# rchikhi/rust-seq2kminmers

Hardware: AMD Instinct MI355X
Metric: input bases/s (Gbp/s) for k-min-mer extraction, l=31 k=10 d=0.01 (higher is better)
Workload: dtype u32

## Files before the change

### rust-seq2kminmers_amd/csrc/s2k_tile_impl.h

```cpp
#pragma once
#include "s2k_dev.h"
#include "s2k_static_l.h"

#include <cstdlib>
#include <mutex>
#include <type_traits>

namespace s2k {
namespace {

#ifndef S2K_TW
#define S2K_TW 12
#endif
#ifndef S2K_TW_REG
#ifdef S2K_PROFILE
#define S2K_TW_REG 12
#else
#define S2K_TW_REG 16
#endif
#endif
template <bool HPC> constexpr int tw() { return HPC ? S2K_TW : S2K_TW_REG; }
template <bool HPC> constexpr int waves_per_simd() { return tw<HPC>() / 4; }
static_assert(S2K_TW % 4 == 0 && S2K_TW_REG % 4 == 0, "whole waves per SIMD");
constexpr int HS_OFF = 16;
constexpr int BUF_BYTES = HS_OFF + TILE_BASES + 128;
#ifndef S2K_CAPP
#define S2K_CAPP 16
#endif
constexpr int CAPP = S2K_CAPP;
constexpr int NPC = TILE_T / CAPP;
constexpr int MAX_L_TILED = 64;
#ifndef S2K_LISTCAP
#define S2K_LISTCAP 256
#endif
#ifndef S2K_JOBCAP
#define S2K_JOBCAP 32
#endif
#ifndef S2K_REDERIVE_GROUP
#define S2K_REDERIVE_GROUP 8
#endif
constexpr int LISTCAP_REG = S2K_TW_REG > 12 ? 216 : S2K_LISTCAP;
constexpr int LISTCAP_HPC = 192;
template <bool HPC> constexpr int listcap() { return HPC ? LISTCAP_HPC : LISTCAP_REG; }
template <bool HPC> constexpr int jobcap() { return !HPC && S2K_TW_REG > 12 ? 16 : S2K_JOBCAP; }
#ifndef S2K_REG_LA
#define S2K_REG_LA 1
#endif
#ifndef S2K_HPC_LA
#define S2K_HPC_LA 2
#endif
constexpr int REG_LA = S2K_REG_LA;
constexpr int HPC_LA = S2K_HPC_LA;
constexpr int NBL = 32;
template <bool DESC> constexpr int stores_per_round() { return DESC ? 1 : 3; }
static_assert(NBL == META_SEGS, "TileMeta keeps NBL segment starts");
constexpr int NPRE = 10;

#ifndef S2K_SD_SHIFT
#define S2K_SD_SHIFT 6
#endif
constexpr int ROW_W = 6, ROW_PFX = 4, ROW_CUM = 5, N_ROWS = 66, SD_SHIFT = S2K_SD_SHIFT;
struct HpcLds {
    uint32_t row[N_ROWS][ROW_W];
    uint32_t halo_pos[64];
    uint8_t sd[SD_SHIFT == 6 ? 160 : 288];
};
static_assert(sizeof(HpcLds) % 16 == 0, "the tile buffer behind it is read 16 bytes at a time");
struct NoHpcLds {};

template <bool HPC>
struct alignas(16) WaveLdsT : std::conditional<HPC, HpcLds, NoHpcLds>::type {
    uint8_t buf[BUF_BYTES];
    uint16_t list[listcap<HPC>()];
    uint16_t jobx[jobcap<HPC>()];
    uint16_t jobslot[jobcap<HPC>()];
    int16_t hb[NBL];
    uint16_t rs16[NBL];
};
#ifdef S2K_PROFILE
typedef __attribute__((address_space(3))) unsigned long long *ph_ptr_t;
constexpr int PROFILE_LDS_BYTES = 16 * 16 * 8;
#else
typedef uint64_t *ph_ptr_t;
constexpr int PROFILE_LDS_BYTES = 0;
#endif
constexpr int SEED_TABLE_BYTES = 2 * 256 * 8;
#ifndef S2K_SEL8
#define S2K_SEL8 1
#endif
constexpr int TABLE_BYTES = SEED_TABLE_BYTES;
constexpr int SEL8_OFF = SEED_TABLE_BYTES, SEL8_BYTES = S2K_SEL8 ? 256 * 8 : 0;
#ifndef S2K_PASS2_ACC
#define S2K_PASS2_ACC 1
#endif
static_assert(!S2K_PASS2_ACC || S2K_SEL8, "pass 2 reads its v_perm_b32 selectors from sel8");
#ifndef S2K_LPH
#define S2K_LPH 0
#endif
#ifndef S2K_WARM2
#define S2K_WARM2 1
#endif
constexpr int WARM_OFF = SEL8_OFF + SEL8_BYTES, WARM_BYTES = S2K_WARM2 ? 256 * 8 : 0;
template <bool HPC> constexpr int table_bytes() { return SEED_TABLE_BYTES + (HPC ? SEL8_BYTES + WARM_BYTES : 0); }
template <bool HPC>
constexpr int block_lds_bytes() { return table_bytes<HPC>() + tw<HPC>() * (int)sizeof(WaveLdsT<HPC>) + PROFILE_LDS_BYTES; }
#ifndef S2K_EXPERIMENT
static_assert(block_lds_bytes<true>() <= 160 * 1024 && block_lds_bytes<false>() <= 160 * 1024, "the block of a CU must fit its 160 KiB of LDS");
#endif

__device__ inline uint32_t wave_incl_scan(uint32_t v, int lane) {
    (void)lane;
    uint32_t t;
    t = (uint32_t)__builtin_amdgcn_update_dpp(0, (int)v, 0x111, 0xf, 0xf, false);
    uint32_t a = v + t;
    t = (uint32_t)__builtin_amdgcn_update_dpp(0, (int)v, 0x112, 0xf, 0xf, false);
    a += t;
    t = (uint32_t)__builtin_amdgcn_update_dpp(0, (int)v, 0x113, 0xf, 0xf, false);
    a += t;
    t = (uint32_t)__builtin_amdgcn_update_dpp(0, (int)a, 0x114, 0xf, 0xe, false);
    a += t;
    t = (uint32_t)__builtin_amdgcn_update_dpp(0, (int)a, 0x118, 0xf, 0xc, false);
    a += t;
// ... 320 lines not shown
#ifdef S2K_ISA_MARKS
#define S2K_STAMP(i) do { (void)ph; (void)stamp; asm volatile("; S2K_PHASE %0" ::"i"(i)); } while (0)
#else
#define S2K_STAMP(i) do { (void)ph; (void)stamp; } while (0)
#endif
#endif

template <class WL>
__device__ __forceinline__ uint32_t hpc_compact(uint8_t *D, WL &S, const uint8_t *__restrict__ bases,
                                                const uint64_t *__restrict__ read_off, uint64_t n_reads, uint64_t n_bases,
                                                uint64_t t0, uint32_t tile_len, uint32_t r0, uint32_t r1, uint32_t l,
                                                int lane, uint32_t &halo_n_out, uint64_t bpos0,
                                                uint32_t prev_byte0, bool forced0, const Sem &sem, ph_ptr_t ph,
                                                uint64_t &stamp) {
    typedef __attribute__((address_space(3))) uint8_t lds_u8;
    {
        uint64_t sp = bpos0;
        for (uint64_t c0 = 0;; c0 += 64) {
            if (sp > t0 && sp < t0 + tile_len) {
                const uint32_t rel = (uint32_t)(sp - t0), o = div_tile_t(rel), i = rel - __umul24(o, (uint32_t)TILE_T);
                atomicOr(&S.row[o][i >> 5], 1u << (i & 31u));
            }
            if ((uint64_t)r0 + 1 + c0 + 64 > (uint64_t)r1) break;
            const uint64_t ri = (uint64_t)r0 + 1 + c0 + 64 + lane;
            sp = ri <= n_reads ? read_off[ri] : ~0ull;
            __builtin_amdgcn_s_waitcnt(0x0F70);
        }
    }
    wave_sync();
    S2K_STAMP(13);
    uint32_t c[36];
    const uint32_t lane_off = __umul24((uint32_t)TILE_T, (uint32_t)lane);
    const uint4 *src = reinterpret_cast<const uint4 *>(D + lane_off);
#pragma unroll
    for (int p = 0; p < 9; p++) {
        uint4 v = src[p];
        c[4 * p] = v.x; c[4 * p + 1] = v.y; c[4 * p + 2] = v.z; c[4 * p + 3] = v.w;
    }
    uint32_t fmk[5];
    {
        const uint2 *rr = reinterpret_cast<const uint2 *>(&S.row[lane][0]);
        const uint2 r01 = rr[0], r23 = rr[1];
        fmk[0] = r01.x; fmk[1] = r01.y; fmk[2] = r23.x; fmk[3] = r23.y;
        fmk[4] = S.row[lane][4];
    }
    if (lane == 0 && forced0) fmk[0] |= 1u;
    const uint32_t prevw = (uint32_t)__builtin_amdgcn_update_dpp((int)(prev_byte0 << 24), (int)c[35], 0x138, 0xf, 0xf, false);
    const uint32_t last_raw = bcast(c[35] >> 24, 63);
    const uint32_t la_a = D[TILE_BASES + lane], la_b = D[TILE_BASES + 64 + lane];
    const int vb = (int)tile_len - (int)lane_off;
    const bool partial = tile_len < (uint32_t)TILE_BASES;
    uint32_t pr[4];
#pragma unroll
    for (int d = 0; d < 36; d++) {
        const uint32_t cur = c[d];
        const uint32_t prv = __builtin_amdgcn_alignbyte(cur, d == 0 ? prevw : c[d - 1], 3);
        uint32_t x;
        asm("v_bitop3_b32 %0, %1, %2, %3 bitop3:0x96" : "=v"(x) : "v"(cur), "v"(prv), "v"(0x0C0C0C0Cu));
        const uint32_t y = __builtin_amdgcn_perm(0xFFFFFFFFu, 0xFFFFFFFFu, x);
        const int j = (d & 7) >> 1;
        if ((d & 1) == 0) pr[j] = __builtin_amdgcn_udot4(y, 0x08040201u, 255u, false);
        else pr[j] = __builtin_amdgcn_udot4(y, 0x80402010u, pr[j], false);
        if (d == 35) fmk[4] |= __builtin_amdgcn_perm(pr[1], pr[0], 0x0C0C0501u);
        else if ((d & 7) == 7)
            fmk[d >> 3] |= __builtin_amdgcn_perm(pr[1], pr[0], 0x0C0C0501u) | __builtin_amdgcn_perm(pr[3], pr[2], 0x05010C0Cu);
    }
    if (partial) {
#pragma unroll
        for (int g = 0; g < 5; g++) {
            const int v = vb - 32 * g;
            fmk[g] &= v >= 32 ? 0xFFFFFFFFu : (v <= 0 ? 0u : ((1u << v) - 1u));
        }
    }
    const uint32_t p0 = __popc(fmk[0]), p1 = p0 + __popc(fmk[1]), p2 = p1 + __popc(fmk[2]), p3 = p2 + __popc(fmk[3]);
    uint32_t cnt = p3 + __popc(fmk[4]);
    uint32_t incl = wave_incl_scan(cnt, lane);
    uint32_t base = incl - cnt;
    const uint32_t R = bcast(incl, 63);
    {
        uint2 *rw = reinterpret_cast<uint2 *>(&S.row[lane][0]);
        rw[0] = make_uint2(fmk[0], fmk[1]);
        rw[1] = make_uint2(fmk[2], fmk[3]);
        rw[2] = make_uint2(fmk[4] | (base << 16), p0 | (p1 << 8) | (p2 << 16) | (p3 << 24));
        if (lane < N_ROWS - 64) *reinterpret_cast<uint2 *>(&S.row[64 + lane][ROW_PFX]) = make_uint2(R << 16, 0u);
        if (cnt)
            for (uint32_t m = (base + (1u << SD_SHIFT) - 1u) >> SD_SHIFT; (m << SD_SHIFT) < base + cnt; m++) S.sd[m] = (uint8_t)lane;
    }
    wave_sync();
    S2K_STAMP(14);
#if S2K_PASS2_ACC
    {
        typedef __attribute__((address_space(3))) const unsigned long long *lds_cu64;
        uint4 *zp = reinterpret_cast<uint4 *>(D + lane_off);
#pragma unroll
        for (int p = 0; p < 9; p++) zp[p] = make_uint4(0, 0, 0, 0);
        asm volatile("" ::: "memory");
        const uint32_t(&fmk_)[5] = fmk;
        auto pass2 = [&](auto sparse_c) {
            constexpr bool SPARSE = decltype(sparse_c)::value;
            uint32_t fm[5] = {fmk_[0], fmk_[1], fmk_[2], fmk_[3], fmk_[4]};
#pragma unroll
            for (int g = 0; g < 5; g++) asm volatile("" : "+v"(fm[g]));
            if constexpr (!SPARSE) {
                uint32_t qa = (uint32_t)(uintptr_t)(lds_u8 *)D + base - 1u, carry = 0;
#pragma unroll
                for (int q0 = 0; q0 < 18; q0 += 9) {
                    unsigned long long e[9];
                    uint32_t ix[9];
#pragma unroll
                    for (int qq = 0; qq < 9; qq++) {
                        ix[qq] = byte_x8_sel(fm[(q0 + qq) >> 2], (q0 + qq) & 3);
                        e[qq] = *reinterpret_cast<lds_cu64>((uint32_t)SEL8_OFF + ix[qq]);
                    }
#pragma unroll
                    for (int qq = 0; qq < 9; qq++) {
                        const int q = q0 + qq;
                        const uint32_t plo = __builtin_amdgcn_perm(c[2 * q + 1], c[2 * q], (uint32_t)e[qq]);
                        const uint32_t phi = __builtin_amdgcn_perm(c[2 * q + 1], c[2 * q], (uint32_t)(e[qq] >> 32));
                        const uint32_t sh = ~qa, waddr = qa & ~3u;
                        const uint32_t w0 = __builtin_amdgcn_alignbyte(plo, 0u, sh) | carry, w1 = __builtin_amdgcn_alignbyte(phi, plo, sh);
                        carry = __builtin_amdgcn_alignbyte(0u, phi, sh);
                        asm volatile("ds_or_b32 %0, %1\n\tds_or_b32 %0, %2 offset:4" ::"v"(waddr), "v"(w0), "v"(w1) : "memory");
                        qa += (uint32_t)__popc(ix[qq]);
                    }
                }
                asm volatile("ds_or_b32 %0, %1" ::"v"(qa & ~3u), "v"(carry) : "memory");
                return;
            }
            uint32_t waddr = (uint32_t)(uintptr_t)(lds_u8 *)D + (base & ~3u);
            uint32_t fill8 = 8u * (base & 3u), lo = 0;
            const uint32_t dump = (uint32_t)(uintptr_t)(lds_u8 *)reinterpret_cast<uint8_t *>(&S.list[0]) + 8u * ((uint32_t)lane & 31u);
            constexpr int GRPQ = 9;
#pragma unroll
            for (int q0 = 0; q0 < 18; q0 += GRPQ) {
                unsigned long long e[GRPQ];
                uint32_t ix[GRPQ];
#pragma unroll
                for (int qq = 0; qq < GRPQ; qq++) {
                    const int q = q0 + qq;
                    ix[qq] = byte_x8_sel(fm[q >> 2], q & 3);
                    e[qq] = *reinterpret_cast<lds_cu64>((uint32_t)SEL8_OFF + ix[qq]);
                }
#pragma unroll
                for (int qq = 0; qq < GRPQ; qq++) {
                    const int q = q0 + qq;
                    const uint32_t plo = __builtin_amdgcn_perm(c[2 * q + 1], c[2 * q], (uint32_t)e[qq]);
                    const uint32_t phi = __builtin_amdgcn_perm(c[2 * q + 1], c[2 * q], (uint32_t)(e[qq] >> 32));
                    const unsigned long long win = (((unsigned long long)phi << 32) | plo) << fill8;
                    const uint32_t w0 = lo | (uint32_t)win, w1 = (uint32_t)(win >> 32);
                    const uint32_t w2 = (phi >> 8) >> (24u - fill8);
                    const uint32_t nb = fill8 + 8u * (uint32_t)__popc(ix[qq]);
                    const uint32_t a0 = nb >= 32u ? waddr : dump, a1 = nb >= 64u ? waddr : dump;
                    asm volatile("ds_write_b32 %0, %2\n\tds_write_b32 %1, %3 offset:4" ::"v"(a0), "v"(a1), "v"(w0), "v"(w1) : "memory");
                    lo = nb >= 64u ? w2 : (nb >= 32u ? w1 : w0);
                    waddr += (nb >> 3) & 0xCu;
                    fill8 = nb & 24u;
                }
            }
            asm volatile("ds_or_b32 %0, %1" ::"v"(waddr), "v"(lo) : "memory");
        };
        static_assert(sizeof(S.list) >= 32 * 8, "the dump slots of the sparse variant live in the hit list");
        if (10u * R < 6u * tile_len) pass2(std::true_type{});
        else pass2(std::false_type{});
    }
#else
    {
        uint32_t gaddr = (uint32_t)(uintptr_t)(lds_u8 *)D + base - 1;
// ... 22 lines not shown
    }
#endif
    S2K_STAMP(15);
    const uint32_t hl = sem.tail_quirk ? l + 16 : l;
    uint32_t halo_n = 0;
    if (!partial) {
        uint32_t pb = last_raw;
#pragma unroll
        for (int rnd = 0; rnd < 2; rnd++) {
            const uint64_t qr = t0 + TILE_BASES + 64 * rnd;
            if (halo_n >= hl || qr >= n_bases) break;
            const uint32_t by = rnd ? la_b : la_a;
            const uint32_t pv = (uint32_t)__builtin_amdgcn_update_dpp((int)pb, (int)by, 0x138, 0xf, 0xf, false);
            const bool hd = qr + (uint64_t)lane < n_bases && by != pv;
            const uint64_t mk = __ballot(hd);
            const uint32_t idx = halo_n + __builtin_amdgcn_mbcnt_hi((uint32_t)(mk >> 32), __builtin_amdgcn_mbcnt_lo((uint32_t)mk, 0u));
            if (hd && idx < hl) {
                D[R + idx] = (uint8_t)by;
                S.halo_pos[idx] = (uint32_t)(TILE_BASES + 64 * rnd) + (uint32_t)lane;
            }
            halo_n += (uint32_t)__popcll(mk);
            pb = bcast(by, 63);
        }
        uint64_t q = t0 + TILE_BASES + 128;
        while (halo_n < hl && q < n_bases) {
            const uint32_t span = 256u;
            uint64_t a = q + 4 * (uint64_t)lane;
            int nval = a >= n_bases ? 0 : (n_bases - a >= 4 ? 4 : (int)(n_bases - a));
            uint32_t wv = 0;
            if (nval == 4) wv = *reinterpret_cast<const uint32_t *>(bases + a);
            else
                for (int b = 0; b < nval; b++) wv |= (uint32_t)bases[a + b] << (8 * b);
            uint32_t pw = __shfl_up(wv, 1);
            if (lane == 0) pw = pb << 24;
            uint32_t prv = (wv << 8) | (pw >> 24);
            uint32_t x = wv ^ prv;
            uint32_t t = (((x & 0x7F7F7F7Fu) + 0x7F7F7F7Fu) | x) & 0x80808080u;
            t &= nval >= 4 ? 0xFFFFFFFFu : (nval <= 0 ? 0u : ((1u << (8 * nval)) - 1u));
            uint32_t cn = __popc(t);
            uint32_t in2 = wave_incl_scan(cn, lane);
            uint32_t idx = halo_n + in2 - cn;
#pragma unroll
            for (int b = 0; b < 4; b++) {
                if (t & (0x80u << (8 * b))) {
                    if (idx < hl) {
                        D[R + idx] = (uint8_t)(wv >> (8 * b));
                        S.halo_pos[idx] = (uint32_t)(a - t0) + b;
                    }
                    idx++;
                }
            }
            halo_n += bcast(in2, 63);
            pb = bcast(wv >> 24, 63);
            q += span;
        }
        if (halo_n > hl) halo_n = hl;
    }
    halo_n_out = halo_n;
    wave_sync();
    return R;
}


struct BmFirst {
    uint32_t x, yy, ox0, oy0, he;
    bool y_in;
};
template <class WL>
__device__ __forceinline__ BmFirst hpc_rawpos_first(const WL &S, uint32_t x, uint32_t l, uint32_t R, uint32_t halo_n) {
    typedef __attribute__((address_space(3))) const uint8_t *lds_cu8;
    BmFirst f;
    const uint32_t y = x + l;
    f.x = x;
    f.y_in = y < R;
    f.yy = f.y_in ? y : x;
    const uint32_t hx = y - R;
    f.he = S.halo_pos[(!f.y_in && hx < halo_n) ? hx : 0];
    const uint32_t sd0 = (uint32_t)(uintptr_t)(lds_cu8)&S.sd[0];
    f.ox0 = reinterpret_cast<lds_cu8>(sd0)[x >> SD_SHIFT];
    f.oy0 = reinterpret_cast<lds_cu8>(sd0)[f.yy >> SD_SHIFT];
    return f;
}
template <class WL>
__device__ __forceinline__ void hpc_rawpos_rest(const WL &S, const BmFirst &f, uint32_t &raw_x, uint32_t &raw_e) {
    typedef __attribute__((address_space(3))) const uint8_t *lds_cu8;
    const uint32_t x = f.x, yy = f.yy, ox0 = f.ox0, oy0 = f.oy0, he = f.he;
    const bool y_in = f.y_in;
    const uint32_t row0 = (uint32_t)(uintptr_t)(lds_cu8)&S.row[0][0];
    typedef __attribute__((address_space(3))) const unsigned long long *lds_cu64;
    typedef __attribute__((address_space(3))) const uint32_t *lds_cu32;
    auto ld2 = [](uint32_t a) {
        const unsigned long long v = *reinterpret_cast<lds_cu64>(a);
        return make_uint2((uint32_t)v, (uint32_t)(v >> 32));
    };
    const uint32_t rx = mad24(ox0, 4u * ROW_W, row0), ry = mad24(oy0, 4u * ROW_W, row0);
    const uint2 ax = ld2(rx + 4 * ROW_PFX), bx = ld2(rx + 4 * (ROW_PFX + ROW_W)), cx = ld2(rx + 4 * (ROW_PFX + 2 * ROW_W));
    const uint2 ay = ld2(ry + 4 * ROW_PFX), by = ld2(ry + 4 * (ROW_PFX + ROW_W)), cy = ld2(ry + 4 * (ROW_PFX + 2 * ROW_W));
    const bool sx = (bx.x >> 16) <= x, sy = (by.x >> 16) <= yy;
    uint32_t rox = sx ? rx + 4 * ROW_W : rx, roy = sy ? ry + 4 * ROW_W : ry;
    uint2 px = sx ? bx : ax, py = sy ? by : ay;
    if (__ballot((cx.x >> 16) <= x || (cy.x >> 16) <= yy)) {
        while ((*reinterpret_cast<lds_cu32>(rox + 4 * (ROW_PFX + ROW_W)) >> 16) <= x) rox += 4 * ROW_W;
        while ((*reinterpret_cast<lds_cu32>(roy + 4 * (ROW_PFX + ROW_W)) >> 16) <= yy) roy += 4 * ROW_W;
        px = ld2(rox + 4 * ROW_PFX);
        py = ld2(roy + 4 * ROW_PFX);
    }
    const uint32_t nx = x - (px.x >> 16), ny = yy - (py.x >> 16);
    const uint32_t gx = word_of_head(px.y, nx), gy = word_of_head(py.y, ny);
    const uint32_t wx = *reinterpret_cast<lds_cu32>(rox + 4u * gx), wy = *reinterpret_cast<lds_cu32>(roy + 4u * gy);
    const uint32_t bx_ = select_nth_32_lut(wx, nx - heads_before_word(px.y, gx)), by_ = select_nth_32_lut(wy, ny - heads_before_word(py.y, gy));
    raw_x = (rox - row0) * (uint32_t)(TILE_T / (4 * ROW_W)) + 32u * gx + bx_;
    const uint32_t re = (roy - row0) * (uint32_t)(TILE_T / (4 * ROW_W)) + 32u * gy + by_;
    raw_e = y_in ? re : he;
}
template <class WL>
__device__ __forceinline__ void hpc_rawpos2(const WL &S, uint32_t x, uint32_t l, uint32_t R, uint32_t halo_n,
                                            uint32_t Tq, uint32_t rcpTq, uint32_t &raw_x, uint32_t &raw_e) {
    (void)Tq;
    (void)rcpTq;
    const BmFirst f = hpc_rawpos_first(S, x, l, R, halo_n);
    hpc_rawpos_rest(S, f, raw_x, raw_e);
}
static_assert(TILE_T % (4 * ROW_W) == 0, "raw offset of a lane = its row offset times a whole number");
template <class WL>
__device__ __forceinline__ uint32_t heads_before_raw(const WL &S, uint32_t rel) {
    const uint32_t o = div_tile_t(rel), wi = rel - __umul24(o, (uint32_t)TILE_T), g = wi >> 5;
    const uint2 pc = *reinterpret_cast<const uint2 *>(&S.row[o][ROW_PFX]);
    const uint32_t wd = S.row[o][g];
    return (pc.x >> 16) + heads_before_word(pc.y, g) + __popc(wd & ((1u << (wi & 31u)) - 1u));
}

__device__ __forceinline__ uint32_t lookback_heads(const uint32_t *W, uint64_t t, int lane, Counts *counts, uint32_t early, bool &dead) {
    uint32_t sum = 0;
    if (dead) return 0;
    for (uint64_t tb = t;;) {
        const bool exists = tb >= 1 + (uint64_t)lane;
        const uint32_t *p = W + (exists ? tb - 1 - (uint64_t)lane : 0);
        uint32_t w = HW_VALID;
        int fs = 64;
        for (int polls = 0;; polls++) {
            if (exists) w = (polls == 0 && tb == t) ? early : __hip_atomic_load(p, __ATOMIC_RELAXED, __HIP_MEMORY_SCOPE_AGENT);
            const uint64_t valid = __ballot((w & HW_VALID) != 0u);
            const uint64_t stop = __ballot((w & HW_VALID) != 0u && (w & HW_PASS) == 0u);
            fs = stop ? __builtin_ctzll(stop) : 64;
            const uint64_t need = fs >= 63 ? ~0ull : ((2ull << fs) - 1ull);
            if ((valid & need) == need) break;
            const bool anybody = (polls & 63) == 63 && __hip_atomic_load(&counts->need_runs, __ATOMIC_RELAXED, __HIP_MEMORY_SCOPE_AGENT) != 0u;
            if (polls >= 4096 || __builtin_amdgcn_readfirstlane((int)anybody)) {
                if (lane == 0) counts->need_runs = 1;
                dead = true;
                return 0;
            }
            __builtin_amdgcn_s_sleep(16);
        }
        const uint32_t mine = (lane <= fs) ? (w & HW_COUNT) : 0u;
        sum += bcast(wave_incl_scan(mine, lane), 63);
        if (fs < 64) break;
        tb -= 64;
    }
    return sum;
}

template <class WL>
__device__ __forceinline__ void publish_tile_heads(uint32_t *W, uint64_t t, const WL &S, uint32_t nh, uint64_t t0, uint32_t tile_len,
                                                   bool any_start, uint64_t last_start, bool first_begins_here, int lane) {
    uint32_t word;
    if (!any_start) {
        word = HW_VALID | (first_begins_here ? 0u : HW_PASS) | nh;
    } else if (last_start >= t0 + tile_len) {
        word = HW_VALID;
    } else {
        const uint32_t c = heads_before_raw(S, (uint32_t)(last_start - t0));
        word = HW_VALID | (nh - c);
    }
    if (lane == 0) __hip_atomic_store(W + t, word, __ATOMIC_RELAXED, __HIP_MEMORY_SCOPE_AGENT);
}

template <int L, bool HPC, bool DESC, class WL, class IssueNext>
__device__ __forceinline__ uint32_t dense_phase(IssueNext &&issue_next, WL &S, const uint8_t *D, const uint2 *tab,
                                                const uint64_t *__restrict__ read_off, uint64_t n_reads, uint64_t t,
                                                uint64_t t0, uint32_t tile_len, uint32_t nh, uint32_t halo_n,
                                                uint32_t Tq, uint32_t rcpTq, uint32_t l, uint32_t r0, uint32_t r1, uint64_t bpos0,
                                                uint64_t rs0, int lane, const Records &rec, uint64_t *pool_cursor,
                                                uint32_t *mn_cnt, Counts *counts, uint64_t &base, const Sem &sem,
                                                unsigned long long *__restrict__ d_agg, TileMeta *__restrict__ d_meta, uint32_t K1,
                                                const uint32_t (&caps)[NPC], const uint32_t (&raw)[5], uint32_t lb_early,
                                                bool &lb_dead, ph_ptr_t ph, uint64_t &stamp) {
    constexpr int LISTCAP = listcap<HPC>();
    const uint32_t wclr = HPC ? (sem.keep_last ? l - 1 : l) : l - 1;
    const uint32_t tql = __umul24(Tq, (uint32_t)lane);
    uint32_t vm[5];
    {
        int vc = (int)nh - (int)tql;
#pragma unroll
        for (int d = 0; d < 5; d++) {
            vm[d] = raw[d] & bits_below(vc - 32 * d);
        }
    }
    const uint64_t tile_end = t0 + tile_len;
    uint32_t nb = 0;
    const bool many = (r1 - r0) > (uint32_t)(NBL - 2);
    bool ext_at_end = false;
    {
        uint64_t bpos = bpos0;
// ... 49 lines not shown
                            const int lo = hb0 - (int)wclr - 16 - (int)tql, hi = hb0 - (int)wclr - 1 - (int)tql;
                            uint32_t inwin = 0;
                            if (hi >= 0 && lo < (int)Tq) {
#pragma unroll
                                for (int d = 0; d < 5; d++) {
                                    const int a = lo - 32 * d, bnd2 = hi - 32 * d;
                                    if (bnd2 >= 0 && a < 32) {
                                        const uint32_t m_hi = bnd2 >= 31 ? 0xFFFFFFFFu : ((2u << bnd2) - 1u);
                                        const uint32_t m_lo = a <= 0 ? 0xFFFFFFFFu : (0xFFFFFFFFu << a);
                                        inwin |= vm[d] & m_hi & m_lo;
                                    }
                                }
                            }
                            if (__ballot(inwin != 0u)) {
                                const uint32_t carried = lookback_heads(sem.tile_heads, t, lane, counts, lb_early, lb_dead);
                                if (lane == 0) Rr += carried;
                            }
                        }
                        hb_carry = (int32_t)bcast((uint32_t)HB, 63);
                    }
                    if (bnd) {
                        if (bpos - pstart <= (uint64_t)l) {
                            wextra = Rr >= l ? 1u : 0u;
                        } else if (Rr >= l) {
                            const uint32_t sentinel = Rr - l + 1;
                            if (sentinel >= 32 && (sentinel & 15) == 0) wextra = 16;
                        }
                    }
                    chunk_prev = ((uint64_t)bcast((uint32_t)(bpos >> 32), 63) << 32) | bcast((uint32_t)bpos, 63);
                }
            }
            if constexpr (!HPC) {
                pstart = ((uint64_t)__shfl_up((uint32_t)(bpos >> 32), 1) << 32) | __shfl_up((uint32_t)bpos, 1);
                if (lane == 0) pstart = chunk_prev;
                if (sem.tail_quirk && bpos != ~0ull && bpos - pstart > (uint64_t)l) {
                    const uint64_t sentinel = bpos - pstart - l + 1;
                    if (sentinel >= 32 && (sentinel & 15) == 0) wextra = 16;
                }
            }
            uint64_t todo = __ballot(internal) | (em ? (1ull << first_ext) : 0ull);
            while (todo) {
                const int z = __builtin_ctzll(todo);
                todo &= todo - 1;
                const int32_t hbz = (int32_t)bcast((uint32_t)HB, z);
                const int wz = (int)wclr + (int)bcast(wextra, z);
                if (hbz - wz >= (int)nh) continue;
                const int lo = hbz - wz - (int)tql, hi = hbz - 1 - (int)tql;
#pragma unroll
                for (int d = 0; d < 5; d++) vm[d] &= ~(bits_below(hi + 1 - 32 * d) & ~bits_below(lo - 32 * d));
            }
            if constexpr (!HPC) {
                const bool exact = bpos != ~0ull && bpos - pstart == (uint64_t)l && pstart >= t0 && pstart < tile_end;
                uint64_t ex = __ballot(exact);
                while (ex) {
                    const int z = __builtin_ctzll(ex);
                    ex &= ex - 1;
                    const uint32_t hx = bcast((uint32_t)(pstart - t0), z);
                    const int rel = (int)hx - (int)tql;
                    if (rel >= 0 && rel < (int)Tq) {
#pragma unroll
                        for (int d = 0; d < 5; d++)
                            if ((rel >> 5) == d) vm[d] &= ~(1u << (rel & 31));
                    }
                }
                chunk_prev = ((uint64_t)bcast((uint32_t)(bpos >> 32), 63) << 32) | bcast((uint32_t)bpos, 63);
            }
            if (!many && internal && c0 + lane < (uint32_t)(NBL - 1)) {
                S.hb[c0 + lane] = (int16_t)HB;
                S.rs16[c0 + lane + 1] = (uint16_t)(bpos - t0);
            }
            nb += (uint32_t)__popcll(__ballot(internal));
            if (em) {
                const uint64_t ebq = ((uint64_t)bcast((uint32_t)(bpos >> 32), first_ext) << 32) | bcast((uint32_t)bpos, first_ext);
                ext_at_end = ebq == tile_end;
                break;
            }
            const uint64_t ri = (uint64_t)r0 + 1 + c0 + 64 + lane;
            bpos = ri <= n_reads ? read_off[ri] : ~0ull;
            __builtin_amdgcn_s_waitcnt(0x0F70);
        }
    }
    S2K_STAMP(3);
    const uint32_t cnt = __popc(vm[0]) + __popc(vm[1]) + __popc(vm[2]) + __popc(vm[3]) + __popc(vm[4]);
    const uint32_t incl = wave_incl_scan(cnt, lane);
    const uint32_t myoff = incl - cnt;
    const uint32_t N = bcast(incl, 63);
    base = t * rec.slab_cap;
    bool dropped = false;
    if (N > rec.slab_cap) {
        uint64_t got = 0;
        if (lane == 0) got = atomicAdd(rec.ovf_cursor, (unsigned long long)N);
        got = ((uint64_t)bcast((uint32_t)(got >> 32), 0) << 32) | bcast((uint32_t)got, 0);
        base = rec.ovf_base + got;
        if (base + N > rec.capacity) {
            if (lane == 0) {
                counts->pool_overflow = 1;
                atomicMax((unsigned long long *)&counts->pool_needed, (unsigned long long)(got + N));
            }
            base = 0;
            dropped = true;
        }
    }
    if constexpr (!DESC) {
        if (N == 0 || dropped) {
            issue_next(0u, base);
            return 0;
        }
    }
    uint32_t mine = 0, segstart = 0;
    if (!many) {
        uint32_t below_prev = 0;
        for (uint32_t i = 0; i <= nb; i++) {
            uint32_t below = N;
            if (i < nb) {
                const int lim = S.hb[i] - (int)tql;
                uint32_t c = 0;
#pragma unroll
                for (int d = 0; d < 5; d++) {
                    c += __popc(vm[d] & bits_below(lim - 32 * d));
                }
                const int hbi = S.hb[i];
                const int lb = hbi <= 0 ? 0 : ((uint32_t)hbi >= Tq * 64u ? 63 : (int)div_tq((uint32_t)hbi, rcpTq));
                below = bcast(myoff + c, lb);
            }
            if ((uint32_t)lane == i) {
                mine = below - below_prev;
                segstart = below_prev;
            }
            below_prev = below;
        }
        if constexpr (!DESC)
            if ((uint32_t)lane <= nb && mine) atomicAdd(&mn_cnt[r0 + lane], mine);
    }
    if constexpr (DESC) {
        if (many) {
            if (lane == 0) counts->need_legacy = 1;
            issue_next(0u, base);
            return 0;
        }
        const bool dep = !(t0 == 0 || rs0 == t0);
        const uint32_t m_first = bcast(mine, 0), m_last = bcast(mine, (int)nb);
        uint32_t wfix = (uint32_t)lane <= nb && mine > K1 ? mine - K1 : 0u;
        if (lane == 0 && dep) wfix = 0;
        uint32_t Cfix;
        if (nb <= 2u) Cfix = bcast(wfix, 0) + (nb >= 1u ? bcast(wfix, 1) : 0u) + (nb >= 2u ? bcast(wfix, 2) : 0u);
        else Cfix = bcast(wave_incl_scan(wfix, lane), 63);
        const bool pass = dep && nb == 0 && !ext_at_end;
        const uint32_t q_out = ext_at_end ? 0u : (m_last < K1 ? m_last : K1);
        if (lane == 0) {
            d_agg[t] = agg_pack(m_first, Cfix, dropped ? 0u : N, q_out, dep, pass);
            TileMeta *m = &d_meta[t];
            m->rec_base = base;
            m->rs0 = rs0;
            m->r0 = r0;
            m->nb = (uint16_t)nb;
            m->nrd = (uint16_t)(r1 - r0);
        }
        if ((uint32_t)lane <= nb) {
            d_meta[t].segstart[lane] = (uint16_t)segstart;
            if (lane) d_meta[t].rs16[lane] = S.rs16[lane];
        }
        if (N == 0 || dropped || (sem.dbg_skip & 128)) {
            issue_next(0u, base);
            return 0;
        }
    }
    uint32_t njobs = 0;
    auto flush_jobs = [&]() {
        wave_sync();
        const uint32_t part = (uint32_t)lane & 3u;
        const uint32_t per = (l + 3u) >> 2;
        const uint32_t i0 = per * part;
        for (uint32_t j0 = 0; j0 < njobs; j0 += 16) {
            const uint32_t job = j0 + ((uint32_t)lane >> 2);
            const bool act = job < njobs;
            const uint8_t *q = D + (act ? S.jobx[job] : 0) + i0;
            uint32_t f = 0, r = 0;
            if constexpr (L > 0) {
                constexpr uint32_t PER = (L + 3) / 4;
                constexpr uint32_t GRP = S2K_REDERIVE_GROUP;
#pragma unroll
                for (uint32_t h0 = 0; h0 < PER; h0 += GRP) {
                    uint32_t by[GRP];
                    uint2 ti[GRP];
#pragma unroll
                    for (uint32_t ii = 0; ii < GRP; ii++)
                        if (h0 + ii < PER) by[ii] = q[h0 + ii];
#pragma unroll
                    for (uint32_t ii = 0; ii < GRP; ii++)
                        if (h0 + ii < PER) ti[ii] = tab_in(tab, by[ii]);
                    uint32_t tf[GRP], tr[GRP];
#pragma unroll
                    for (uint32_t ii = 0; ii < GRP; ii++) {
                        tf[ii] = tr[ii] = 0u;
                        if (h0 + ii < PER) {
                            const uint32_t i = i0 + h0 + ii, rot = (uint32_t)L - 1u - i;
                            const bool valid = 3 * PER + h0 + ii < (uint32_t)L || i < (uint32_t)L;
                            tf[ii] = valid ? rotl32(ti[ii].x, rot) : 0u;
                            tr[ii] = valid ? rotr32(ti[ii].y, rot) : 0u;
                        }
                    }
#pragma unroll
                    for (uint32_t ii = 0; ii < GRP; ii += 4) {
                        f = xor3(xor3(f, tf[ii], tf[ii + 1]), tf[ii + 2], tf[ii + 3]);
                        r = xor3(xor3(r, tr[ii], tr[ii + 1]), tr[ii + 2], tr[ii + 3]);
                    }
                    if (GRP < PER) __builtin_amdgcn_sched_barrier(0);
                }
            } else {
                for (uint32_t ii = 0; ii < per; ii++) {
                    const uint32_t i = i0 + ii;
                    if (i < l) {
                        const uint2 ti = tab_in(tab, q[ii]);
                        f ^= rotl32(ti.x, l - 1 - i);
                        r ^= rotr32(ti.y, l - 1 - i);
                    }
                }
            }
            f ^= (uint32_t)__builtin_amdgcn_update_dpp(0, (int)f, 0xB1, 0xf, 0xf, false);
            r ^= (uint32_t)__builtin_amdgcn_update_dpp(0, (int)r, 0xB1, 0xf, 0xf, false);
            f ^= (uint32_t)__builtin_amdgcn_update_dpp(0, (int)f, 0x4E, 0xf, 0xf, false);
            r ^= (uint32_t)__builtin_amdgcn_update_dpp(0, (int)r, 0x4E, 0xf, 0xf, false);
            if (act && part == 0) rec.hash[base + S.jobslot[job]] = f < r ? f : r;
        }
        njobs = 0;
        wave_sync();
    };
    auto batch = [&](uint32_t b0, auto single_c) {
        uint32_t *const rec_j = rec.j, *const rec_hash = rec.hash, *const rec_jend = rec.jend, *const rec_rid = rec.rid;
        constexpr bool SINGLE = decltype(single_c)::value;
        wave_sync();
        bool listed = false;
        if constexpr (HPC && SINGLE && S2K_LPH != 0) {
            if (Tq <= 112u) {
                listed = true;
                typedef __attribute__((address_space(3))) uint8_t lds_b;
                typedef __attribute__((address_space(3))) uint32_t lds_w;
                typedef uint32_t u32x2 __attribute__((ext_vector_type(2)));
                typedef uint32_t u32x4 __attribute__((ext_vector_type(4)));
                typedef __attribute__((address_space(3))) u32x2 lds_w2;
                typedef __attribute__((address_space(3))) u32x4 lds_w4;
                constexpr uint32_t XT = TILE_BASES + 128 - 2048;
                static_assert(XT % 16 == 0 && XT >= 7168 + MAX_L_TILED + 16 && LISTCAP <= 192, "the tables of the listing must not reach into the compacted tile");
                const uint32_t dq = (uint32_t)(uintptr_t)(lds_b *)const_cast<uint8_t *>(D) + XT;
                constexpr uint32_t T2O = 1024, DIRO = 1536;
                if (lane < 12) *reinterpret_cast<lds_w4 *>(dq + DIRO + 16u * (uint32_t)lane) = u32x4{0u, 0u, 0u, 0u};
                *reinterpret_cast<lds_w4 *>(dq + 16u * (uint32_t)lane) = u32x4{vm[0], vm[1], vm[2], vm[3]};
                const uint32_t c0 = __popc(vm[0]), c1 = c0 + __popc(vm[1]), c2 = c1 + __popc(vm[2]);
                uint32_t lp = 0;
#pragma unroll
                for (int pc = 0; pc < 7; pc++) {
                    const uint32_t hw = (pc & 1) ? raw[pc >> 1] >> 16 : raw[pc >> 1] & 0xFFFFu;
                    lp |= (31u - (uint32_t)__builtin_clz(hw | 1u)) << (4 * pc);
                }
                *reinterpret_cast<lds_w2 *>(dq + T2O + 8u * (uint32_t)lane) = u32x2{c0 | (c1 << 8) | (c2 << 16) | (myoff << 24), lp};
                if (cnt) *reinterpret_cast<lds_b *>(dq + DIRO + myoff) = (uint8_t)(lane + 1);
                wave_sync();
                uint32_t own[3] = {0, 0, 0};
                uint32_t carry = 0;
#pragma unroll
                for (int rd = 0; rd < 3; rd++) {
                    if (64u * rd < N) {
                        const uint32_t kq = 64u * rd + (uint32_t)lane;
                        const bool act = kq < N;
                        uint32_t dv = act ? (uint32_t)*reinterpret_cast<lds_b *>(dq + DIRO + kq) : 0u;
                        dv = wave_incl_max(dv);
                        dv = dv > carry ? dv : carry;
                        carry = bcast(dv, 63);
                        const uint32_t o = act ? dv - 1u : 0u;
                        const u32x2 t2 = *reinterpret_cast<lds_w2 *>(dq + T2O + 8u * o);
                        const uint32_t n = kq - (t2.x >> 24);
                        uint32_t g = 0;
                        asm("v_cmp_ge_u32_sdwa vcc, %1, %2 src0_sel:DWORD src1_sel:BYTE_0\n\t"
                            "v_addc_co_u32_e32 %0, vcc, 0, %0, vcc\n\t"
                            "v_cmp_ge_u32_sdwa vcc, %1, %2 src0_sel:DWORD src1_sel:BYTE_1\n\t"
                            "v_addc_co_u32_e32 %0, vcc, 0, %0, vcc\n\t"
                            "v_cmp_ge_u32_sdwa vcc, %1, %2 src0_sel:DWORD src1_sel:BYTE_2\n\t"
                            "v_addc_co_u32_e32 %0, vcc, 0, %0, vcc"
                            : "+v"(g)
                            : "v"(n), "v"(t2.x)
                            : "vcc");
                        if (!act) g = 0;
                        const uint32_t hbw = heads_before_word(t2.x, g);
                        const uint32_t wv = *reinterpret_cast<lds_w *>(dq + 16u * o + 4u * g);
                        const uint32_t ps = 32u * g + select_nth_32_lut(wv, act ? n - hbw : 0u);
                        const uint32_t piece = ps >> 4;
                        const bool later = ((t2.y >> (4u * piece)) & 15u) != (ps & 15u);
                        if (act) S.list[kq] = (uint16_t)((__umul24(Tq, o) + ps) | (later ? 0x8000u : 0u));
                        own[rd] = o | (piece << 8) | (later || !act ? 0x8000u : 0u);
                    }
                }
                wave_sync();
#pragma unroll
                for (int pc = 0; pc < 7; pc++) *reinterpret_cast<lds_w *>(dq + 256u * pc + 4u * (uint32_t)lane) = caps[pc];
                wave_sync();
#pragma unroll
                for (int rd = 0; rd < 3; rd++) {
                    if (64u * rd < N && !(sem.dbg_skip & 16)) {
                        if (!(own[rd] & 0x8000u))
                            rec.hash[base + 64u * rd + (uint32_t)lane] = *reinterpret_cast<lds_w *>(dq + 256u * ((own[rd] >> 8) & 15u) + 4u * (own[rd] & 0xFFu));
                    }
                }
            }
        }
        if (!listed) {
            uint32_t k = myoff;
#pragma unroll
            for (int d = 0; d < 5; d++) {
                uint32_t wv = vm[d];
                const uint32_t rw = raw[d];
                constexpr int CPW = 32 / CAPP;
                auto capw = [&](int i) { return caps[(CPW * d + i) < NPC ? CPW * d + i : NPC - 1]; };
                const uint32_t cap0 = capw(0), cap1 = capw(1), cap2 = capw(CPW > 2 ? 2 : 0), cap3 = capw(CPW > 2 ? 3 : 1);
                while (wv) {
                    const uint32_t bit = __builtin_ctz(wv);
                    wv &= wv - 1;
                    const uint32_t pm = CAPP == 16 ? (0xFFFFu << (bit & 16)) : (0xFFu << (bit & 24));
                    const uint32_t later = rw & (pm & ~((2u << bit) - 1u));
                    const uint32_t hvk = CAPP == 16 ? ((bit & 16) ? cap1 : cap0) : ((bit & 16) ? ((bit & 8) ? cap3 : cap2) : ((bit & 8) ? cap1 : cap0));
                    if (SINGLE || (k >= b0 && k < b0 + LISTCAP)) {
                        S.list[k - b0] = (uint16_t)((tql + 32 * d + bit) | (later ? 0x8000u : 0u));
                        if (!later && !(sem.dbg_skip & 16)) rec_hash[base + k] = hvk;
                    }
                    k++;
                }
            }
        }
        wave_sync();
        S2K_STAMP(4);
        const uint32_t bn = N - b0 < (uint32_t)LISTCAP ? N - b0 : (uint32_t)LISTCAP;
        for (uint32_t k0 = 0; k0 < bn; k0 += 64) {
            const uint32_t kq = k0 + lane;
            const uint32_t e = kq < bn ? S.list[kq] : 0u;
            const bool need = (e & 0x8000u) != 0;
            uint64_t jobs = __ballot(need);
#ifdef S2K_PROFILE
            if ((sem.dbg_skip & 8) && lane == 0) ph[7] += (uint64_t)__popcll(jobs);
#endif
            if (sem.dbg_skip & 64) jobs = 0;
            while (jobs) {
                const uint32_t room = (uint32_t)jobcap<HPC>() - njobs;
                const uint32_t rank = (uint32_t)__popcll(jobs & ((1ull << lane) - 1ull));
                const bool minej = need && ((jobs >> lane) & 1ull) && rank < room;
                if (minej) {
                    S.jobx[njobs + rank] = (uint16_t)(e & 0x3FFFu);
                    S.jobslot[njobs + rank] = (uint16_t)(b0 + kq);
                }
                const uint64_t done = __ballot(minej);
                njobs += (uint32_t)__popcll(done);
                jobs &= ~done;
                if (jobs) flush_jobs();
            }
        }
        if (njobs) flush_jobs();
        S2K_STAMP(12);
        if (b0 + (uint32_t)LISTCAP >= N) issue_next(N, base);
        auto backmap = [&](uint32_t x, uint32_t &p, uint32_t &e1) {
            if constexpr (HPC) {
                uint32_t rp = 0, re = 0;
                const uint32_t back = sem.end_kind == 2 ? 1u : 0u;
                hpc_rawpos2(S, x, l - back, nh, halo_n, Tq, rcpTq, rp, re);
                e1 = re - (1u - back);
                p = rp;
            } else {
                p = x;
                e1 = x + l - 1;
            }
        };
        auto rounds = [&](auto many_c) {
        constexpr bool MANY = decltype(many_c)::value;
        for (uint32_t k0 = 0; k0 < bn; k0 += 64) {
            asm volatile("; S2K_MARK round_begin many=%0" ::"i"(MANY ? 1 : 0));
            const uint32_t kk = k0 + lane;
            const bool act = kk < bn;
            uint32_t x = 0, rid = 0;
            uint32_t prel = 0, erel = 0;
            if (act) x = S.list[kk] & 0x3FFFu;
            S2K_STAMP(8);
            if (act) backmap(x, prel, erel);
            S2K_STAMP(9);
            if constexpr (DESC) {
                if (act) {
                    const uint32_t span = erel - prel;
                    if (span > (uint32_t)REC_SPAN_MAX) counts->need_legacy = 1;
                    const uint32_t sp = span > (uint32_t)REC_SPAN_MAX ? (uint32_t)REC_SPAN_MAX : span;
                    if (!(sem.dbg_skip & 16)) rec_j[base + b0 + kk] = prel | (sp << 14);
                }
            } else {
            const uint64_t p = t0 + prel, e1 = t0 + erel;
            if (act) {
                uint64_t rstart;
                if constexpr (!MANY) {
                    uint32_t c = 0;
                    for (uint32_t i = 0; i < nb; i++) c += (S.hb[i] <= (int32_t)x);
                    rid = r0 + c;
                    rstart = c == 0 ? rs0 : t0 + S.rs16[c];
                } else {
                    uint32_t lo = r0, hi = r1;
                    while (lo < hi) {
                        uint32_t mid = lo + (hi - lo + 1) / 2;
                        if (read_off[mid] <= p) lo = mid;
                        else hi = mid - 1;
                    }
                    rid = lo;
                    rstart = read_off[lo];
                }
                const uint64_t slot = base + b0 + kk;
                if (!(sem.dbg_skip & 16)) {
                    rec_j[slot] = (uint32_t)(p - rstart);
                    rec_jend[slot] = (uint32_t)(e1 - rstart);
                    rec_rid[slot] = rid;
                }
            }
            S2K_STAMP(10);
            if constexpr (MANY) {
                uint64_t remm = __ballot(act);
                while (remm) {
                    const int z = __builtin_ctzll(remm);
                    const uint32_t rz = bcast(rid, z);
                    const uint64_t same = __ballot(act && rid == rz);
                    if (lane == z) atomicAdd(&mn_cnt[rz], (uint32_t)__popcll(same));
                    remm &= ~same;
                }
            }
            }
            asm volatile("; S2K_MARK round_end many=%0" ::"i"(MANY ? 1 : 0));
        }
        };
        if constexpr (DESC) {
            rounds(std::false_type{});
        } else {
            if (many) rounds(std::true_type{});
            else rounds(std::false_type{});
        }
    };
    if (N <= (uint32_t)LISTCAP) batch(0u, std::true_type{});
    else
        for (uint32_t b0 = 0; b0 < N; b0 += LISTCAP) batch(b0, std::false_type{});
    return N;
}

template <int MODE>
__device__ __forceinline__ Sem tile_sem(Sem s) {
#ifndef S2K_DEBUG_KNOBS
    s.dbg_skip = 0;
#endif
    if constexpr (MODE != TILE_MODE_RUNTIME) {
        s.enabled = 1;
        s.hpc = MODE == TILE_MODE_HPC;
        s.simd_seeds = 0;
        s.keep_last = MODE == TILE_MODE_HPC ? 0 : 1;
// ... 593 lines not shown
```

Before: 1881.

## Rederive job hashes with lane-parallel Horner and skip third-row probe when dense

Adds a new flush_jobs path for HPC with fixed L that computes each rederive job's hash cooperatively, using two or four lanes per job. Each lane runs a Horner-style rolling of seeds over its chunk, and the partial hashes are combined with DPP xor shuffles. This replaces the older per-part loop. The tile-build step now stores a wave-wide sparse flag in the padding row, and backmap skips the third prefix-row loads and walk unless some lane had fewer than 64 heads. The job-queue loop is also restructured so the final flush is folded into the per-chunk loop, and some record pointers are hoisted later. Risks: correctness of the combine and rotation maths depends on L and the split, and the flag's meaning relies on the density assumption.

Measured after the change: 1900 (median of 6 runs). No clear change (+1.0%).

```diff
diff --git a/rust-seq2kminmers_amd/csrc/s2k_tile_impl.h b/rust-seq2kminmers_amd/csrc/s2k_tile_impl.h
--- a/rust-seq2kminmers_amd/csrc/s2k_tile_impl.h
+++ b/rust-seq2kminmers_amd/csrc/s2k_tile_impl.h
@@ -38,6 +38,12 @@
 #endif
 #ifndef S2K_REDERIVE_GROUP
 #define S2K_REDERIVE_GROUP 8
+#endif
+#ifndef S2K_REDERIVE_HORNER
+#define S2K_REDERIVE_HORNER 1
+#endif
+#ifndef S2K_ROW3_LAZY
+#define S2K_ROW3_LAZY 1
 #endif
 constexpr int LISTCAP_REG = S2K_TW_REG > 12 ? 216 : S2K_LISTCAP;
 constexpr int LISTCAP_HPC = 192;
@@ -524,7 +530,8 @@
         rw[0] = make_uint2(fmk[0], fmk[1]);
         rw[1] = make_uint2(fmk[2], fmk[3]);
         rw[2] = make_uint2(fmk[4] | (base << 16), p0 | (p1 << 8) | (p2 << 16) | (p3 << 24));
-        if (lane < N_ROWS - 64) *reinterpret_cast<uint2 *>(&S.row[64 + lane][ROW_PFX]) = make_uint2(R << 16, 0u);
+        const uint32_t sparse = __ballot(cnt < 64u) != 0ull ? 1u : 0u;
+        if (lane < N_ROWS - 64) *reinterpret_cast<uint2 *>(&S.row[64 + lane][ROW_PFX]) = make_uint2(R << 16, sparse);
         if (cnt)
             for (uint32_t m = (base + (1u << SD_SHIFT) - 1u) >> SD_SHIFT; (m << SD_SHIFT) < base + cnt; m++) S.sd[m] = (uint8_t)lane;
     }
@@ -713,7 +720,7 @@
     return f;
 }
 template <class WL>
-__device__ __forceinline__ void hpc_rawpos_rest(const WL &S, const BmFirst &f, uint32_t &raw_x, uint32_t &raw_e) {
+__device__ __forceinline__ void hpc_rawpos_rest(const WL &S, const BmFirst &f, bool sparse, uint32_t &raw_x, uint32_t &raw_e) {
     typedef __attribute__((address_space(3))) const uint8_t *lds_cu8;
     const uint32_t x = f.x, yy = f.yy, ox0 = f.ox0, oy0 = f.oy0, he = f.he;
     const bool y_in = f.y_in;
@@ -725,12 +732,12 @@
         return make_uint2((uint32_t)v, (uint32_t)(v >> 32));
     };
     const uint32_t rx = mad24(ox0, 4u * ROW_W, row0), ry = mad24(oy0, 4u * ROW_W, row0);
-    const uint2 ax = ld2(rx + 4 * ROW_PFX), bx = ld2(rx + 4 * (ROW_PFX + ROW_W)), cx = ld2(rx + 4 * (ROW_PFX + 2 * ROW_W));
-    const uint2 ay = ld2(ry + 4 * ROW_PFX), by = ld2(ry + 4 * (ROW_PFX + ROW_W)), cy = ld2(ry + 4 * (ROW_PFX + 2 * ROW_W));
+    const uint2 ax = ld2(rx + 4 * ROW_PFX), bx = ld2(rx + 4 * (ROW_PFX + ROW_W));
+    const uint2 ay = ld2(ry + 4 * ROW_PFX), by = ld2(ry + 4 * (ROW_PFX + ROW_W));
     const bool sx = (bx.x >> 16) <= x, sy = (by.x >> 16) <= yy;
     uint32_t rox = sx ? rx + 4 * ROW_W : rx, roy = sy ? ry + 4 * ROW_W : ry;
     uint2 px = sx ? bx : ax, py = sy ? by : ay;
-    if (__ballot((cx.x >> 16) <= x || (cy.x >> 16) <= yy)) {
+    if (sparse && __ballot((ld2(rx + 4 * (ROW_PFX + 2 * ROW_W)).x >> 16) <= x || (ld2(ry + 4 * (ROW_PFX + 2 * ROW_W)).x >> 16) <= yy)) {
         while ((*reinterpret_cast<lds_cu32>(rox + 4 * (ROW_PFX + ROW_W)) >> 16) <= x) rox += 4 * ROW_W;
         while ((*reinterpret_cast<lds_cu32>(roy + 4 * (ROW_PFX + ROW_W)) >> 16) <= yy) roy += 4 * ROW_W;
         px = ld2(rox + 4 * ROW_PFX);
@@ -746,11 +753,11 @@
 }
 template <class WL>
 __device__ __forceinline__ void hpc_rawpos2(const WL &S, uint32_t x, uint32_t l, uint32_t R, uint32_t halo_n,
-                                            uint32_t Tq, uint32_t rcpTq, uint32_t &raw_x, uint32_t &raw_e) {
+                                            uint32_t Tq, uint32_t rcpTq, bool sparse, uint32_t &raw_x, uint32_t &raw_e) {
     (void)Tq;
     (void)rcpTq;
     const BmFirst f = hpc_rawpos_first(S, x, l, R, halo_n);
-    hpc_rawpos_rest(S, f, raw_x, raw_e);
+    hpc_rawpos_rest(S, f, sparse, raw_x, raw_e);
 }
 static_assert(TILE_T % (4 * ROW_W) == 0, "raw offset of a lane = its row offset times a whole number");
 template <class WL>
@@ -1052,6 +1059,60 @@
     uint32_t njobs = 0;
     auto flush_jobs = [&]() {
         wave_sync();
+        if constexpr (L > 0 && HPC && S2K_WARM2 != 0 && S2K_REDERIVE_HORNER != 0) {
+            static_assert(jobcap<HPC>() <= 32, "two lanes per job: 32 jobs fill the wave");
+            constexpr uint32_t LL = (uint32_t)L, C = (LL + 3u) / 4u, NDW = (C + 3u) / 4u;
+            typedef __attribute__((address_space(3))) const uint8_t lds_cu8;
+            typedef __attribute__((address_space(3))) const uint32_t lds_cu32;
+            uint32_t sft = njobs > 16u ? 1u : 2u;
+            asm volatile("" : "+v"(sft));
+            const uint32_t job = (uint32_t)lane >> sft, part = (uint32_t)lane & ((1u << sft) - 1u);
+            uint32_t i0 = C * (part << (2u - sft));
+            uint32_t a = (uint32_t)(uintptr_t)(lds_cu8 *)&S.buf[HS_OFF] + (uint32_t)S.jobx[job < njobs ? job : njobs - 1u] + i0;
+            uint32_t f = 0, r = 0;
+            for (uint32_t h = njobs > 16u ? 2u : 1u; h; h--, a += C, i0 += C) {
+                uint32_t w[NDW + 1], v[NDW];
+#pragma unroll
+                for (uint32_t d = 0; d <= NDW; d++) w[d] = *reinterpret_cast<lds_cu32 *>((a & ~3u) + 4u * d);
+#pragma unroll
+                for (uint32_t d = 0; d < NDW; d++) v[d] = __builtin_amdgcn_alignbyte(w[d + 1], w[d], a);
+                uint2 E[C];
+#pragma unroll
+                for (uint32_t jj = 0; jj < C; jj++) {
+                    const uint32_t off = byte_x8_sel(v[jj >> 2], (int)(jj & 3u));
+                    E[jj] = (jj % 2u == 0u && jj + 1u < C) ? seed_pair<WARM_OFF>(off) : seed_pair<0>(off);
+                }
+#pragma unroll
+                for (uint32_t jj = 0; jj < C; jj++)
+                    if (3u * C + jj >= LL) {
+                        const uint32_t valid = (uint32_t)((int32_t)(i0 + jj - LL) >> 31);
+                        E[jj].x &= valid;
+                        E[jj].y &= valid;
+                    }
+#pragma unroll
+                for (uint32_t jj = 0; jj + 1u < C; jj += 2) {
+                    f = xor3(__builtin_rotateleft32(f, 2), E[jj].x, E[jj + 1].x);
+                    r = xor3(__builtin_rotateright32(r, 2), E[jj].y, E[jj + 1].y);
+                }
+                if constexpr (C % 2u == 1u) {
+                    f = __builtin_rotateleft32(f, 1) ^ E[C - 1].x;
+                    r = __builtin_rotateright32(r, 1) ^ E[C - 1].y;
+                }
+            }
+            const uint32_t sh = (LL - i0) & 31u;
+            f = __builtin_rotateleft32(f, sh);
+            r = __builtin_rotateright32(r, sh);
+            f ^= (uint32_t)__builtin_amdgcn_update_dpp(0, (int)f, 0xB1, 0xf, 0xf, false);
+            r ^= (uint32_t)__builtin_amdgcn_update_dpp(0, (int)r, 0xB1, 0xf, 0xf, false);
+            if (njobs <= 16u) {
+                f ^= (uint32_t)__builtin_amdgcn_update_dpp(0, (int)f, 0x4E, 0xf, 0xf, false);
+                r ^= (uint32_t)__builtin_amdgcn_update_dpp(0, (int)r, 0x4E, 0xf, 0xf, false);
+            }
+            if (job < njobs && part == 0) rec.hash[base + S.jobslot[job]] = f < r ? f : r;
+            njobs = 0;
+            wave_sync();
+            return;
+        }
         const uint32_t part = (uint32_t)lane & 3u;
         const uint32_t per = (l + 3u) >> 2;
         const uint32_t i0 = per * part;
@@ -1111,7 +1172,7 @@
         wave_sync();
     };
     auto batch = [&](uint32_t b0, auto single_c) {
-        uint32_t *const rec_j = rec.j, *const rec_hash = rec.hash, *const rec_jend = rec.jend, *const rec_rid = rec.rid;
+        uint32_t *const rec_hash = rec.hash;
         constexpr bool SINGLE = decltype(single_c)::value;
         wave_sync();
         bool listed = false;
@@ -1216,34 +1277,40 @@
         for (uint32_t k0 = 0; k0 < bn; k0 += 64) {
             const uint32_t kq = k0 + lane;
             const uint32_t e = kq < bn ? S.list[kq] : 0u;
-            const bool need = (e & 0x8000u) != 0;
-            uint64_t jobs = __ballot(need);
+            uint32_t rederive = e >> 15;
+            asm volatile("" : "+v"(rederive));
+            uint64_t jobs = __ballot(rederive != 0u);
 #ifdef S2K_PROFILE
             if ((sem.dbg_skip & 8) && lane == 0) ph[7] += (uint64_t)__popcll(jobs);
 #endif
             if (sem.dbg_skip & 64) jobs = 0;
-            while (jobs) {
-                const uint32_t room = (uint32_t)jobcap<HPC>() - njobs;
-                const uint32_t rank = (uint32_t)__popcll(jobs & ((1ull << lane) - 1ull));
-                const bool minej = need && ((jobs >> lane) & 1ull) && rank < room;
-                if (minej) {
-                    S.jobx[njobs + rank] = (uint16_t)(e & 0x3FFFu);
-                    S.jobslot[njobs + rank] = (uint16_t)(b0 + kq);
-                }
-                const uint64_t done = __ballot(minej);
-                njobs += (uint32_t)__popcll(done);
-                jobs &= ~done;
-                if (jobs) flush_jobs();
-            }
-        }
-        if (njobs) flush_jobs();
+            do {
+                if (jobs) {
+                    const uint32_t room = (uint32_t)jobcap<HPC>() - njobs;
+                    const uint32_t rank = (uint32_t)__popcll(jobs & ((1ull << lane) - 1ull));
+                    const bool minej = ((jobs >> lane) & 1ull) && rank < room;
+                    if (minej) {
+                        S.jobx[njobs + rank] = (uint16_t)(e & 0x3FFFu);
+                        S.jobslot[njobs + rank] = (uint16_t)(b0 + kq);
+                    }
+                    const uint64_t done = __ballot(minej);
+                    njobs += (uint32_t)__popcll(done);
+                    jobs &= ~done;
+                }
+                uint32_t kn = k0 + 64u;
+                asm volatile("" : "+s"(kn));
+                if (jobs || (njobs && kn >= bn)) flush_jobs();
+            } while (jobs);
+        }
         S2K_STAMP(12);
         if (b0 + (uint32_t)LISTCAP >= N) issue_next(N, base);
+        bool sparse = true;
+        if constexpr (HPC && S2K_ROW3_LAZY != 0) sparse = __builtin_amdgcn_readfirstlane((int)S.row[64][ROW_CUM]) != 0;
         auto backmap = [&](uint32_t x, uint32_t &p, uint32_t &e1) {
             if constexpr (HPC) {
                 uint32_t rp = 0, re = 0;
                 const uint32_t back = sem.end_kind == 2 ? 1u : 0u;
-                hpc_rawpos2(S, x, l - back, nh, halo_n, Tq, rcpTq, rp, re);
+                hpc_rawpos2(S, x, l - back, nh, halo_n, Tq, rcpTq, sparse, rp, re);
                 e1 = re - (1u - back);
                 p = rp;
             } else {
@@ -1251,6 +1318,7 @@
                 e1 = x + l - 1;
             }
         };
+        uint32_t *const rec_j = rec.j, *const rec_jend = rec.jend, *const rec_rid = rec.rid;
         auto rounds = [&](auto many_c) {
         constexpr bool MANY = decltype(many_c)::value;
         for (uint32_t k0 = 0; k0 < bn; k0 += 64) {
```

## Build job queue directly during list emission using packed flag-count scan

Applied to the files above, without the earlier changes.

Packs the count of flagged (non-final-in-piece) minimizer positions into the upper half of the existing wave prefix scan. In the single-pass case this lets each lane write list entries and job queue entries directly at precomputed offsets while emitting. The separate ballot-and-compact pass that rescans the list to gather jobs is then skipped whenever the flagged count fits in the job capacity. This adds per-piece ballot loops and bit-reverse work, and it assumes the counts fit in 16 bits.

After: 1882 before, 1881 after. About the same (-0.1%).

```diff
diff --git a/rust-seq2kminmers_amd/csrc/s2k_tile_impl.h b/rust-seq2kminmers_amd/csrc/s2k_tile_impl.h
--- a/rust-seq2kminmers_amd/csrc/s2k_tile_impl.h
+++ b/rust-seq2kminmers_amd/csrc/s2k_tile_impl.h
@@ -966,9 +966,28 @@
     }
     S2K_STAMP(3);
     const uint32_t cnt = __popc(vm[0]) + __popc(vm[1]) + __popc(vm[2]) + __popc(vm[3]) + __popc(vm[4]);
-    const uint32_t incl = wave_incl_scan(cnt, lane);
+    constexpr bool PIECES = CAPP == 16;
+    uint32_t keep[5] = {0u, 0u, 0u, 0u, 0u};
+    uint32_t nflag = 0;
+    if constexpr (PIECES) {
+        uint32_t nkeep = 0;
+#pragma unroll
+        for (int d = 0; d < 5; d++) {
+            if (d < 4 || Tq > 128u) {
+                const uint32_t rr = __builtin_bitreverse32(raw[d]);
+                const uint32_t rlo = rr >> 16;
+                const uint32_t top = __builtin_bitreverse32((rr & (0u - rr)) | ((rlo & (0u - rlo)) << 16));
+                keep[d] = vm[d] & top;
+                nkeep += __popc(keep[d]);
+            }
+        }
+        nflag = cnt - nkeep;
+    }
+    const uint32_t incl2 = wave_incl_scan(PIECES ? cnt | (nflag << 16) : cnt, lane);
+    const uint32_t incl = PIECES ? incl2 & 0xFFFFu : incl2;
     const uint32_t myoff = incl - cnt;
     const uint32_t N = bcast(incl, 63);
+    const uint32_t flagend = incl2 >> 16;
     base = t * rec.slab_cap;
     bool dropped = false;
     if (N > rec.slab_cap) {
@@ -1187,6 +1206,54 @@
                 }
             }
         }
+        bool queued = false;
+        uint32_t qn = 0;
+        if constexpr (PIECES && SINGLE) {
+            if (!listed) {
+                listed = true;
+                const uint32_t nflag_tile = bcast(flagend, 63);
+                const bool direct = nflag_tile <= (uint32_t)jobcap<HPC>() && !(sem.dbg_skip & 64);
+                uint32_t run = myoff, jq = flagend;
+#pragma unroll
+                for (int g = 0; g < NPC; g++) {
+                    const int d = g >> 1;
+                    const uint32_t v = (g & 1) ? vm[d] >> 16 : vm[d] << 16;
+                    if (__ballot(v != 0u)) {
+                        const uint32_t kv = (g & 1) ? keep[d] >> 16 : keep[d] << 16;
+                        uint32_t f = v ^ kv;
+                        const uint32_t x0 = tql + 32 * d + ((g & 1) ? 16 : -16);
+                        run += __popc(v);
+                        uint32_t rk = run;
+                        if (kv) {
+                            rk--;
+                            S.list[rk] = (uint16_t)(x0 + (31u - (uint32_t)__builtin_clz(kv)));
+                            if (!(sem.dbg_skip & 16)) rec_hash[base + rk] = caps[g];
+                        }
+                        auto flagged_step = [&]() {
+                            if (f) {
+                                const uint32_t bit = 31u - (uint32_t)__builtin_clz(f);
+                                f ^= 1u << bit;
+                                rk--;
+                                S.list[rk] = (uint16_t)((x0 + bit) | 0x8000u);
+                                if (direct) {
+                                    jq--;
+                                    S.jobx[jq] = (uint16_t)(x0 + bit);
+                                    S.jobslot[jq] = (uint16_t)rk;
+                                }
+                            }
+                        };
+                        while (__ballot(f != 0u)) flagged_step();
+                    }
+                }
+                if (direct) {
+#ifdef S2K_PROFILE
+                    if ((sem.dbg_skip & 8) && lane == 0) ph[7] += (uint64_t)nflag_tile;
+#endif
+                    queued = true;
+                    qn = nflag_tile;
+                }
+            }
+        }
         if (!listed) {
             uint32_t k = myoff;
 #pragma unroll
@@ -1213,6 +1280,8 @@
         wave_sync();
         S2K_STAMP(4);
         const uint32_t bn = N - b0 < (uint32_t)LISTCAP ? N - b0 : (uint32_t)LISTCAP;
+        if (queued) njobs = qn;
+        else
         for (uint32_t k0 = 0; k0 < bn; k0 += 64) {
             const uint32_t kq = k0 + lane;
             const uint32_t e = kq < bn ? S.list[kq] : 0u;
```
